# pengsongyou/openscene

Measured on AMD Instinct MI355X. Metric: active voxels/sec MinkUNet18A fwd+bwd @2cm ScanNet; per-point query ms, higher is better.
Workload: dtype f32 (bf16x6 split-precision MFMA, fp32 accumulate); 1 GPU; ScanNet distillation step (configs[2]): MinkUNet18A, 768-d head, 1 synthetic S100k scene/GPU (100999 voxels on rank 0, 2 cm), training-mode BN; timed = coordinate+kernel maps, forward, cosine loss, backward, gradient all-reduce, Adam step; arch=MinkUNet18A, feature_dim=768, voxels_rank0=100999, parallelism=dp1

## Files before the change

### include/openscene_amd.h

```cpp
#ifndef OPENSCENE_AMD_H
#define OPENSCENE_AMD_H

#include <stddef.h>
#include <stdint.h>

#ifdef __cplusplus
extern "C" {
#endif

#define OSN_OK 0
#define OSN_E_ARG (-1)
#define OSN_E_HIP (-2)
#define OSN_E_WS (-3)
#define OSN_E_RANGE (-4)

typedef void* osn_stream_t;

int osn_version(void);
const char* osn_last_error(void);
int osn_device_ok(void);

int64_t osn_hash_capacity(int64_t n);
size_t osn_coords_unique_ws_bytes(int64_t n);

// ... 60 lines not shown
int osn_spconv_fwd_tl_pc(const float* in, int64_t n_in, const void* Wp, const void* tl, const int32_t* out_rows,
                         float* out, double* bn_partial, int64_t n_out, int K, int cin, int cout, int bm,
                         void* ws, size_t ws_bytes, int32_t* counters, osn_stream_t stream);

enum { OSN_PREP_X6 = 0, OSN_PREP_TL = 1 };
typedef struct osn_prep_job {
    const float* W;
    void* out;
    int64_t first_block;
    int32_t K, cin, cout;
    int32_t flip;
    int32_t for_dgrad;
    int32_t layout;
} osn_prep_job;
int64_t osn_weight_prep_job_blocks(int K, int cin, int cout, int for_dgrad, int layout);
int osn_weight_prep_batch(const osn_prep_job* jobs_dev, int n_jobs, int64_t total_blocks, osn_stream_t stream);

int osn_spconv_fwd_plan(int64_t n_out, int K, int cin, int cout, int32_t* plan6);

int osn_stem_conv_ok(int K, int cin, int cout);
int osn_spconv_fwd_tl_ok(int64_t n_in, int K, int cin, int cout);
int osn_dense_fwd_ok(int cin, int cout);
int osn_spconv_fwd_x6_ok(int64_t n_out, int K, int cin, int cout);

int osn_weight_transpose(const float* W, int K, int cin, int cout, int flip, float* Wt,
                         osn_stream_t stream);

size_t osn_spconv_wgrad_ws_bytes(int64_t n_out, int K, int cin, int cout);
size_t osn_spconv_wgrad_items_bytes(int64_t n_out, int K, int cin, int cout);
int osn_spconv_wgrad_plan(const int64_t* counts, int64_t n_out, int K, int cin, int cout,
                          int32_t* items , osn_stream_t stream);
int osn_spconv_wgrad(const float* in, const float* gout, const int32_t* nbr, const int64_t* counts,
                     const int32_t* plan_items, float* gW, int64_t n_out, int K, int cin, int cout,
                     void* ws, size_t ws_bytes, osn_stream_t stream);

size_t osn_pair_lists_bytes(int64_t n_out, int K, int bm);
int osn_pair_lists_build(const void* tl, const int32_t* out_rows, int64_t n_out, int K, int bm, void* pl,
                         osn_stream_t stream);
size_t osn_spconv_wgrad_tl_ws_bytes(int K, int cin, int cout);
int osn_spconv_wgrad_tl(const float* in, const float* gout, const void* pl, int swap, float* gW, int64_t n_in,
                        int64_t n_out, int K, int cin, int cout, void* ws, size_t ws_bytes, osn_stream_t stream);

typedef struct osn_wgrad_job {
    const float* partial;
    const void* range;
    float* gW;
// ... 386 lines not shown
```

### openscene_amd/_lib.py

```python
import ctypes
import os
import threading

_HERE = os.path.dirname(os.path.abspath(__file__))
LIB_PATH = os.environ.get("OSN_LIB_PATH") or os.path.join(_HERE, "lib", "libopenscene_amd.so")

_c = ctypes
_vp, _i32, _i64, _sz, _f32 = _c.c_void_p, _c.c_int, _c.c_int64, _c.c_size_t, _c.c_float

PROTOTYPES = {
    "osn_version": (_i32, []),
    "osn_last_error": (_c.c_char_p, []),
    "osn_device_ok": (_i32, []),
    "osn_hash_capacity": (_i64, [_i64]),
    "osn_coords_unique_ws_bytes": (_sz, [_i64]),
    "osn_coords_unique": (_i32, [_vp, _i64, _i32, _vp, _vp, _i64, _vp, _vp, _vp, _c.POINTER(_i64), _vp, _sz, _vp]),
    "osn_coords_unique_async": (_i32, [_vp, _i64, _vp, _i32, _vp, _vp, _i64, _vp, _vp, _vp, _vp, _vp, _vp, _sz, _vp]),
    "osn_coords_pyramid_async": (_i32, [_vp, _i64, _vp, _i32, _vp, _vp, _i64, _vp, _vp, _vp, _vp, _vp, _sz, _vp]),
    "osn_kmap_build": (_i32, [_vp, _vp, _i64, _vp, _i64, _i32, _i32, _vp, _vp, _vp]),
    "osn_kmap_build_self": (_i32, [_vp, _vp, _i64, _vp, _i64, _i32, _i32, _vp, _vp, _vp]),
    "osn_kmap_transpose": (_i32, [_vp, _i64, _i32, _i64, _vp, _vp]),
    "osn_kmap_sort_ws_bytes": (_sz, [_i64]),
    "osn_kmap_sort": (_i32, [_vp, _i64, _i32, _vp, _vp, _vp, _vp, _vp, _sz, _vp]),
    "osn_kmap_count": (_i32, [_vp, _i64, _i32, _vp, _vp]),
    "osn_spconv_fwd_ws_bytes": (_sz, [_i64, _i32, _i32, _i32]),
    "osn_spconv_fwd": (_i32, [_vp, _vp, _vp, _vp, _vp, _vp, _i64, _i32, _i32, _i32, _vp, _sz, _vp]),
    "osn_weight_prep_x6_bytes": (_sz, [_i32, _i32, _i32, _i32]),
    "osn_weight_prep_x6": (_i32, [_vp, _i32, _i32, _i32, _i32, _i32, _vp, _vp]),
    "osn_weight_prep_x6_pair": (_i32, [_vp, _i32, _i32, _i32, _i32, _vp, _vp, _vp]),
    "osn_spconv_fwd_x6": (_i32, [_vp, _vp, _vp, _vp, _vp, _vp, _i64, _i32, _i32, _i32, _vp, _sz, _vp]),
    "osn_spconv_fwd_plan": (_i32, [_i64, _i32, _i32, _i32, _c.POINTER(_i32)]),
    "osn_stem_conv_ok": (_i32, [_i32, _i32, _i32]),
    "osn_spconv_fwd_tl_ok": (_i32, [_i64, _i32, _i32, _i32]),
    "osn_dense_fwd_ok": (_i32, [_i32, _i32]),
    "osn_spconv_fwd_x6_ok": (_i32, [_i64, _i32, _i32, _i32]),
    "osn_tile_rows": (_i32, [_i64]),
    "osn_tile_lists_bytes": (_sz, [_i64, _i32, _i32]),
    "osn_tile_lists_build": (_i32, [_vp, _i64, _i32, _i32, _vp, _vp]),
    "osn_weight_prep_tl_bytes": (_sz, [_i32, _i32, _i32, _i32]),
    "osn_weight_prep_tl": (_i32, [_vp, _i32, _i32, _i32, _i32, _vp, _vp, _vp]),
    "osn_weight_prep_job_blocks": (_i64, [_i32, _i32, _i32, _i32, _i32]),
    "osn_weight_prep_batch": (_i32, [_vp, _i32, _i64, _vp]),
    "osn_spconv_fwd_tl_ws_bytes": (_sz, [_i64, _i32, _i32, _i32]),
    "osn_spconv_fwd_tl": (_i32, [_vp, _i64, _vp, _vp, _vp, _vp, _vp, _i64, _i32, _i32, _i32, _i32, _vp, _sz, _vp]),
    "osn_spconv_fwd_tl_pc": (_i32, [_vp, _i64, _vp, _vp, _vp, _vp, _vp, _i64, _i32, _i32, _i32, _i32, _vp, _sz, _vp, _vp]),
    "osn_weight_transpose": (_i32, [_vp, _i32, _i32, _i32, _i32, _vp, _vp]),
    "osn_spconv_wgrad_ws_bytes": (_sz, [_i64, _i32, _i32, _i32]),
    "osn_spconv_wgrad_items_bytes": (_sz, [_i64, _i32, _i32, _i32]),
    "osn_spconv_wgrad_plan": (_i32, [_vp, _i64, _i32, _i32, _i32, _vp, _vp]),
    "osn_spconv_wgrad": (_i32, [_vp, _vp, _vp, _vp, _vp, _vp, _i64, _i32, _i32, _i32, _vp, _sz, _vp]),
    "osn_pair_lists_bytes": (_sz, [_i64, _i32, _i32]),
    "osn_pair_lists_build": (_i32, [_vp, _vp, _i64, _i32, _i32, _vp, _vp]),
    "osn_spconv_wgrad_tl_ws_bytes": (_sz, [_i32, _i32, _i32]),
    "osn_spconv_wgrad_tl": (_i32, [_vp, _vp, _vp, _i32, _vp, _i64, _i64, _i32, _i32, _i32, _vp, _sz, _vp]),
    "osn_distill_loss_state_bytes": (_sz, [_i64, _i64]),
    "osn_distill_loss_fwd": (_i32, [_vp, _vp, _vp, _i64, _i64, _i32, _i32, _vp, _vp, _sz, _vp]),
    "osn_distill_loss_bwd": (_i32, [_vp, _vp, _vp, _i64, _i64, _i32, _i32, _vp, _vp, _sz, _vp]),
    "osn_distill_loss_bwd_rows": (_i32, [_vp, _vp, _vp, _i64, _i64, _i32, _i32, _vp, _vp, _vp, _sz, _vp]),
# ... 171 lines not shown
```

### openscene_amd/csrc/spconv_tl.hip

```cpp
#include "common.h"
#include <atomic>
#include <type_traits>
#include "weight_prep.h"
#include "split.h"
#include "epilogue.h"

namespace osn {

constexpr int TL_BMAX = 88;
constexpr int TL_LIST_BMAX = 128;
constexpr int TL_BMIN = 32;
constexpr int TL_BOCC3 = 64;
constexpr int TL_LCAP = 1024;
constexpr int TL_STEPS = TL_LCAP / 32 * 4;
constexpr int TL_KMAX = 128;
constexpr int TL_CIN_MAX = TL_STEPS / (TL_LCAP / 32) * 128;
constexpr int64_t TL_ROWS_MAX = int64_t(1) << 24;
constexpr int TL_SLOTS = 512;
constexpr int TL_MAX_DEVICES = 64;

struct TlView {
    int32_t* cnt;
    int2* lst;
    int64_t nt;
    size_t bytes;
};

static TlView tl_view(const void* base, int64_t n_out, int K, int bm) {
    TlView v;
    char* p = static_cast<char*>(const_cast<void*>(base));
    v.nt = cdiv(n_out > 0 ? n_out : 1, bm);
    const size_t cb = align_up(size_t(v.nt) * K * 4, 256);
    v.cnt = reinterpret_cast<int32_t*>(p);
    v.lst = reinterpret_cast<int2*>(p ? p + cb : nullptr);
    v.bytes = cb + size_t(v.nt) * K * bm * 8;
    return v;
}

__global__ __launch_bounds__(256) void tile_lists_kernel(const int32_t* __restrict__ nbr, int64_t n_out, int K, int bm,
                                                         int32_t* __restrict__ cnt, int2* __restrict__ lst) {
    const int lane = threadIdx.x & 63, wave = threadIdx.x >> 6;
    const int64_t tile = blockIdx.x;
// ... 24 lines not shown
}

#define TL_TICK(slot)                                              \
    if (PROF) {                                                    \
        __builtin_amdgcn_sched_barrier(0);                         \
        const long long now_ = __builtin_amdgcn_s_memtime();       \
        tacc[slot] += now_ - tlast;                                \
        tlast = now_;                                              \
        __builtin_amdgcn_sched_barrier(0);                         \
    }

template <int NW, int KS, bool RAGGED, bool PROF = false, int OCC = 2, bool BUFG = false, bool EPI = false>
__global__ __launch_bounds__(256, OCC) void spconv_tl_kernel(const float* __restrict__ in, const bf16x8* __restrict__ Wp,
                                                               const int32_t* __restrict__ cnt, const int2* __restrict__ lst,
                                                               const int32_t* __restrict__ out_rows, float* __restrict__ out,
                                                               double* __restrict__ bn_partial, int32_t* __restrict__ counter,
                                                               float* __restrict__ partial, int nz, int n_out, int K, int cin,
                                                               int cout, int bm, int n_tiles, int ns, int ncb,
                                                               int self_reset, long long* __restrict__ prof, unsigned in_bytes,
                                                               const Epi epi) {
    static_assert(!(BUFG && RAGGED), "the buffer gather is for full channel chunks");
    constexpr int NT = 256;
    constexpr int CW = 32 * NW;
    constexpr int S = CW + 4;
    constexpr int CK = 32 * KS;
    constexpr int LDA = CK + 8;
    constexpr int QPR = CK / 4;
    constexpr int NQ = (32 * QPR + NT - 1) / NT;
    constexpr int NL = (TL_LCAP + NT - 1) / NT;
    extern __shared__ __attribute__((aligned(16))) float otile[];
    __shared__ __attribute__((aligned(16))) __bf16 stage[3][32][LDA];
    __shared__ uint32_t plist[TL_LCAP];
    __shared__ int klist[TL_KMAX];
    __shared__ int kcnt[TL_KMAX];
    __shared__ int lstart[TL_KMAX + 1];
    __shared__ unsigned char gowner[TL_LCAP / 32];
    __shared__ uint4 stab[TL_STEPS];
    __shared__ int nact_s, bend_s, tile_s;

    long long tacc[10] = {0, 0, 0, 0, 0, 0, 0, 0, 0, 0};
    long long tlast = PROF ? __builtin_amdgcn_s_memtime() : 0;

    const int tid = threadIdx.x, lane = tid & 63;
    const int wave = __builtin_amdgcn_readfirstlane(tid >> 6);
    const int col0 = blockIdx.y * CW;
    const int cw = wave;
    const int cb0 = blockIdx.y * (2 * NW) + 2 * cw;

    int q_row[NQ], q_col[NQ];
#pragma unroll
    for (int j = 0; j < NQ; ++j) {
        const int idx = tid + NT * j;
        q_row[j] = (idx / QPR) & 31;
        q_col[j] = (idx % QPR) * 4;
    }
    const __amdgpu_buffer_rsrc_t insrc = __builtin_amdgcn_make_buffer_rsrc(const_cast<float*>(in), 0, int(BUFG ? in_bytes : 0u), 0x00020000);
    const unsigned cin4 = unsigned(cin) * 4u;

    bf16x8 B[KS][2][3];
    float4 P0[NQ], P1[NQ];
    constexpr bool ragged = RAGGED;
    uint32_t boff[2];
#pragma unroll
    for (int nb = 0; nb < 2; ++nb) boff[nb] = (cb0 + nb < ncb ? unsigned(cb0 + nb) : 0u) * 1024u + 16u * unsigned(lane);
    const uint32_t plane_bytes = unsigned(K) * unsigned(ns) * unsigned(ncb) * 1024u;
    const uint32_t kstep_bytes = unsigned(ncb) * 1024u;
    const __amdgpu_buffer_rsrc_t wrsrc =
        __builtin_amdgcn_make_buffer_rsrc(const_cast<bf16x8*>(Wp), 0, int(3u * plane_bytes), 0x00020000);

    for (;;) {
        if (tid == 0) tile_s = atomicAdd(&counter[blockIdx.y], 1);
        __syncthreads();
        const int draw = __builtin_amdgcn_readfirstlane(tile_s);
        if (draw >= n_tiles * nz) break;
        const int tile = n_tiles - 1 - draw / nz;
        const int zpart = draw - (draw / nz) * nz;
        const int row0 = tile * bm;
        const int rows = min(bm, n_out - row0);
// ... 133 lines not shown
                }
            };
            bool b_ahead = false;
            auto step = [&](const Step& it, float4 (&P)[NQ], const Step& n1s, const Step& nf) {
                bf16x4 p1[NQ], p2[NQ], p3[NQ];
#pragma unroll
                for (int j = 0; j < NQ; ++j) {
                    float4 v = P[j];
                    if (ragged && !(32 * it.s0() + q_col[j] < cin)) v = make_float4(0.f, 0.f, 0.f, 0.f);
                    tl_split4(v, p1[j], p2[j], p3[j]);
                }
                TL_TICK(2)
                if (it.first() && !b_ahead && cw < NW) {
#pragma unroll
                    for (int ks = 0; ks < KS; ++ks) load_b(ks, it);
                }
                const bool ahead = n1s.valid() && n1s.first() && cw < NW;
                TL_TICK(8)
                __syncthreads();
                TL_TICK(3)
#pragma unroll
                for (int j = 0; j < NQ; ++j) {
                    if (NT * NQ == 32 * QPR || tid + NT * j < 32 * QPR) {
                        *reinterpret_cast<bf16x4*>(&stage[0][q_row[j]][q_col[j]]) = p1[j];
                        *reinterpret_cast<bf16x4*>(&stage[1][q_row[j]][q_col[j]]) = p2[j];
                        *reinterpret_cast<bf16x4*>(&stage[2][q_row[j]][q_col[j]]) = p3[j];
                    }
                }
                if (nf.valid()) fetch(nf, P);
                TL_TICK(9)
                __syncthreads();
                TL_TICK(4)
                if (cw >= NW) { b_ahead = false; return; }
                const bool half1 = it.np() > 16;
                const int pbase = it.base + (lane & 15);
                int ocell[2];
                f32x4 acc[2][2];
#pragma unroll
                for (int h = 0; h < 2; ++h) {
                    if (h == 0 || half1) {
                        ocell[h] = int(plist[pbase + 16 * h] >> 24) * S + 32 * cw + 4 * (lane >> 4);
                        const f32x4* cell = reinterpret_cast<const f32x4*>(__builtin_assume_aligned(&otile[ocell[h]], 16));
#pragma unroll
                        for (int nb = 0; nb < 2; ++nb) acc[h][nb] = cell[4 * nb];
                    }
                }
                const int akq = 8 * (lane >> 4);
#pragma unroll
                for (int ks = 0; ks < KS; ++ks) {
                    if (!ragged || it.s0() + ks < ns) {
                        bf16x8 af[2][3];
#pragma unroll
                        for (int h = 0; h < 2; ++h)
#pragma unroll
                            for (int pl = 0; pl < 3; ++pl)
                                af[h][pl] = *reinterpret_cast<const bf16x8*>(&stage[pl][(half1 ? h : 0) * 16 + (lane & 15)][ks * 32 + akq]);
                        auto mfma_half = [&](int h, auto ap, auto bp) {
#pragma unroll
                            for (int nb = 0; nb < 2; ++nb)
                                acc[h][nb] = __builtin_amdgcn_mfma_f32_16x16x32_bf16(B[ks][nb][bp], af[h][ap], acc[h][nb], 0, 0, 0);
                        };
                        if (half1) split_products([&](auto ap, auto bp) { mfma_half(0, ap, bp); mfma_half(1, ap, bp); });
                        else split_products([&](auto ap, auto bp) { mfma_half(0, ap, bp); });
                    }
                    if (ahead) load_b(ks, n1s);
                }
                b_ahead = ahead;
                if (PROF) {
                    float sink = 0.f;
#pragma unroll
                    for (int h = 0; h < 2; ++h)
#pragma unroll
                        for (int nb = 0; nb < 2; ++nb)
                            if (h == 0 || half1) sink += acc[h][nb][0];
                    asm volatile("" ::"v"(sink));
                }
                TL_TICK(5)
#pragma unroll
                for (int h = 0; h < 2; ++h) {
                    if (h == 0 || half1) {
                        f32x4* cell = reinterpret_cast<f32x4*>(__builtin_assume_aligned(&otile[ocell[h]], 16));
#pragma unroll
                        for (int nb = 0; nb < 2; ++nb) cell[4 * nb] = acc[h][nb];
                    }
                }
                TL_TICK(6)
            };

            Step cur = entry(0), n1 = entry(1), n2 = entry(2);
            int tn = 3;
            if (cur.valid()) fetch(cur, P0);
            if (n1.valid()) fetch(n1, P1);
            while (cur.valid()) {
                step(cur, P0, n1, n2);
                cur = n1; n1 = n2; n2 = entry(tn++);
                if (!cur.valid()) break;
                step(cur, P1, n1, n2);
                cur = n1; n1 = n2; n2 = entry(tn++);
            }
            a0 = a1;
        }
        if (park && tid < rows) orow_s[tid] = orow_pre;
        __syncthreads();

        constexpr int V = CW / 4;
        if constexpr (EPI) {
            constexpr int RPP = NT / V;
            const int c4 = tid % V, col = col0 + 4 * c4;
            if (tid < RPP * V && col < cout) {
                const EpiCols ec = epi_cols(epi, col);
                for (int j = tid / V; j < rows; j += RPP) {
                    const float4 v = *reinterpret_cast<const float4*>(&otile[j * S + 4 * c4]);
                    const int64_t orow = park ? orow_s[j] : (out_rows ? out_rows[row0 + j] : row0 + j);
                    *reinterpret_cast<float4*>(out + orow * cout + col) = epi_apply(epi, ec, v, orow, col, cout);
                }
            }
        } else
        for (int idx = tid; idx < rows * V; idx += NT) {
            const int j = idx / V, c4 = idx - j * V;
            const int col = col0 + 4 * c4;
            if (col < cout) {
                const float4 v = *reinterpret_cast<const float4*>(&otile[j * S + 4 * c4]);
                if (nz > 1) {
                    *reinterpret_cast<float4*>(partial + (int64_t(zpart) * n_out + row0 + j) * cout + col) = v;
                } else {
                    const int64_t orow = park ? orow_s[j] : (out_rows ? out_rows[row0 + j] : row0 + j);
                    *reinterpret_cast<float4*>(out + orow * cout + col) = v;
                }
            }
        }
        if (bn_partial) {
            for (int c = tid; c < CW; c += NT) {
                if (col0 + c < cout) {
                    double s1 = 0, s2 = 0;
                    for (int j = 0; j < rows; ++j) {
                        const double v = otile[j * S + c];
                        s1 += v;
                        s2 += v * v;
                    }
                    bn_partial[(int64_t(tile) * 2 + 0) * cout + col0 + c] = s1;
                    bn_partial[(int64_t(tile) * 2 + 1) * cout + col0 + c] = s2;
                }
            }
        }
        __syncthreads();
        TL_TICK(7)
    }
    if (PROF && tid == 0 && blockIdx.y == 0)
        for (int i = 0; i < 10; ++i) prof[int64_t(blockIdx.x) * 10 + i] = tacc[i];
    if ((self_reset & 1) && tid == 0) {
        const int done = atomicAdd(&counter[64 + blockIdx.y], 1);
        if (done == int(gridDim.x) - 1) {
            counter[blockIdx.y] = 0;
            counter[64 + blockIdx.y] = 0;
        }
    }
}
#undef TL_TICK

// ... 74 lines not shown
    return 512 + (nz > 1 ? size_t(nz) * size_t(n_out) * size_t(cout) * 4 : 0);
}

template <bool EPI>
__global__ void tl_reduce_parts_kernel(const float4* __restrict__ partial, int S, int64_t n_out, int c4,
                                       const int32_t* __restrict__ out_rows, float4* __restrict__ out, const Epi epi) {
    const int64_t total = n_out * c4;
    for (int64_t e = int64_t(blockIdx.x) * blockDim.x + threadIdx.x; e < total; e += int64_t(gridDim.x) * blockDim.x) {
        float4 s = partial[e];
        for (int z = 1; z < S; ++z) {
            const float4 v = partial[int64_t(z) * total + e];
            s.x += v.x; s.y += v.y; s.z += v.z; s.w += v.w;
        }
        const int64_t r = e / c4, c = e - r * c4;
        const int64_t orow = out_rows ? int64_t(out_rows[r]) : r;
        if constexpr (EPI) s = epi_quad(epi, s, orow, int(4 * c), 4 * c4);
        out[orow * c4 + c] = s;
    }
}

extern "C" int osn_spconv_fwd_tl_ok(int64_t n_in, int K, int cin, int cout) {
    return K >= 1 && K <= TL_KMAX && cin >= 8 && cin <= TL_CIN_MAX && (cin & 3) == 0 && cout >= 4 && (cout & 3) == 0 && n_in >= 0 &&
           n_in <= TL_ROWS_MAX;
}

static int spconv_fwd_tl_impl(const float* in, int64_t n_in, const void* Wp, const void* tl, const int32_t* out_rows,
                              float* out, double* bn_partial, int64_t n_out, int K, int cin, int cout, int bm, void* ws,
                              size_t ws_bytes, int32_t* counters, long long* prof, osn_stream_t stream, const Epi& epi = epi_none()) {
    hipStream_t st = static_cast<hipStream_t>(stream);
    OSN_REQUIRE(n_out >= 0 && n_out < (int64_t(1) << 31), OSN_E_ARG, "osn_spconv_fwd_tl: n_out out of range");
    OSN_REQUIRE(K >= 1 && K <= TL_KMAX && cin >= 4 && (cin & 3) == 0 && cout >= 4 && (cout & 3) == 0, OSN_E_ARG,
                "osn_spconv_fwd_tl: needs K <= %d, cin %% 4 == 0, cout %% 4 == 0 (K=%d cin=%d cout=%d)", TL_KMAX, K, cin, cout);
    OSN_REQUIRE(bm >= 1 && bm <= TL_BMAX, OSN_E_ARG, "osn_spconv_fwd_tl: bm=%d (at most %d rows per tile)", bm, TL_BMAX);
    OSN_REQUIRE(n_in >= 0 && n_in <= TL_ROWS_MAX, OSN_E_RANGE,
                "osn_spconv_fwd_tl: %lld input rows (the kernel packs an input row into 24 bits; use osn_spconv_fwd_x6)", (long long)n_in);
    if (n_out == 0) return OSN_OK;
    OSN_REQUIRE(in && Wp && out, OSN_E_ARG, "osn_spconv_fwd_tl: null pointer");
    OSN_REQUIRE(tl || (K == 1 && !out_rows), OSN_E_ARG, "osn_spconv_fwd_tl: tile lists may be null only for K == 1 (identity map)");
    OSN_REQUIRE(aligned16(in) && aligned16(Wp) && aligned16(out), OSN_E_ARG, "osn_spconv_fwd_tl: pointers must be 16-byte aligned");
    const int nw = tl_waves(cout);
    const int gy = int(cdiv(cout, 32 * nw));
    const int nz = tl ? tl_split(n_out, K, cout, bm) : 1;
    const size_t need = osn_spconv_fwd_tl_ws_bytes(n_out, tl ? K : 1, cout, bm);
    OSN_REQUIRE(ws && ws_bytes >= need && gy <= 64, OSN_E_WS, "osn_spconv_fwd_tl: workspace %zu < %zu (or more than 64 column groups)", ws_bytes, need);
    OSN_REQUIRE(!(bn_partial && nz > 1), OSN_E_ARG, "osn_spconv_fwd_tl: bn_partial is not available on split (small-table) launches");
    int32_t* counter = counters;
// ... 2 lines not shown
        counter = static_cast<int32_t*>(ws);
    }
    const int self_reset = counters ? 1 : 0;
    float* partial = reinterpret_cast<float*>(static_cast<char*>(ws) + 512);
    const int32_t* cnt = nullptr;
    const int2* lst = nullptr;
    const int64_t n_tiles = cdiv(n_out, bm);
    if (tl) {
        TlView v = tl_view(tl, n_out, K, bm);
        cnt = v.cnt; lst = v.lst;
    }
    const int ns = (cin + 31) / 32, ncb = (cout + 15) / 16;
    const int64_t units = n_tiles * nz;
    unsigned gx = unsigned(units < TL_SLOTS ? units : TL_SLOTS);
    dim3 grid(gx, unsigned(gy));
    const bf16x8* wp = static_cast<const bf16x8*>(Wp);
    const int ks = ns <= 4 ? ns : (ns % 4 == 0 ? 4 : (ns % 3 == 0 ? 3 : 4));
    OSN_REQUIRE(cdiv(ns, ks) * (TL_LCAP / 32) <= TL_STEPS, OSN_E_RANGE,
                "osn_spconv_fwd_tl: %d input channels need more than %d channel chunks per list batch (the kernel's step table); "
                "use osn_dense_fwd (K == 1) or osn_spconv_fwd_x6", cin, TL_STEPS / (TL_LCAP / 32));
    const bool ragged = (cin & 31) != 0 || ns % ks != 0;
    const bool ragged_host = ragged;
    const int ks_host = ks;
    const size_t tile_bytes = size_t(bm + 1) * size_t(32 * nw + 4) * 4;
    const bool occ3 = !prof && !ragged_host && nw <= 3 && ks_host <= 3 && tile_bytes + 28 * 1024 <= 54 * 1024;
    const uint64_t in_bytes64 = uint64_t(n_in) * uint64_t(cin) * 4u;
    const bool bufg = !prof && !ragged_host && in_bytes64 < (uint64_t(1) << 31) && n_in < (int64_t(1) << 24) && int64_t(4) * cin < (int64_t(1) << 24);
    const unsigned in_bytes = bufg ? unsigned(in_bytes64) : 0u;
    int rc_attr = OSN_OK;
    int dev_id = 0;
    OSN_HIP(hipGetDevice(&dev_id));
    const bool dev_slot_ok = dev_id >= 0 && dev_id < TL_MAX_DEVICES;
    const int dev_slot = dev_slot_ok ? dev_id : 0;
    if (occ3) {
        gx = unsigned(units < TL_SLOTS / 2 * 3 ? units : TL_SLOTS / 2 * 3);
        grid = dim3(gx, unsigned(gy));
    }
    const bool use_epi = epi.mean != nullptr && nz == 1;
#define OSN_TL4(NW_, KS_, RG_, PF_, OC_) OSN_TL5(NW_, KS_, RG_, PF_, OC_, false)
#define OSN_TL5(NW_, KS_, RG_, PF_, OC_, BG_)                                                                              \
    do {                                                                                                                   \
        if (use_epi) OSN_TL6(NW_, KS_, RG_, PF_, OC_, BG_, true);                                                          \
        else OSN_TL6(NW_, KS_, RG_, PF_, OC_, BG_, false);                                                                 \
    } while (0)
#define OSN_TL6(NW_, KS_, RG_, PF_, OC_, BG_, EP_)                                                                         \
    do {                                                                                                                   \
        auto kern = spconv_tl_kernel<NW_, KS_, RG_, PF_, OC_, BG_, EP_>;                                                   \
               \
        static std::atomic<unsigned char> attr_set[TL_MAX_DEVICES];                                                        \
        if (tile_bytes > 36 * 1024 && !(dev_slot_ok && attr_set[dev_slot].load(std::memory_order_relaxed))) {              \
            if (hipFuncSetAttribute(reinterpret_cast<const void*>(kern), hipFuncAttributeMaxDynamicSharedMemorySize,       \
                                    int(size_t(TL_BMAX + 1) * size_t(32 * NW_ + 4) * 4)) != hipSuccess) {                  \
                rc_attr = OSN_E_HIP;                                                                                       \
                break;                                                                                                     \
            }                                                                                                              \
            if (dev_slot_ok) attr_set[dev_slot].store(1, std::memory_order_relaxed);                                       \
        }                                                                                                                  \
        hipLaunchKernelGGL(kern, grid, dim3(256), tile_bytes, st, in, wp, cnt, lst, out_rows, out, bn_partial, counter, partial, nz, \
                           int(n_out), K, cin, cout, bm, int(n_tiles), ns, ncb, self_reset, prof, in_bytes,                \
                           use_epi ? epi : epi_none());                                                                    \
    } while (0)
#define OSN_TL3(NW_, KS_, RG_, PF_) OSN_TL4(NW_, KS_, RG_, PF_, 2)
#define OSN_TL2(NW_, KS_)                                                                                                  \
    do {                                                                                                                   \
        if (prof) {                                                                                                        \
            if (ragged) OSN_TL3(NW_, KS_, true, true);                                                                     \
            else OSN_TL3(NW_, KS_, false, true);                                                                           \
        } else if (ragged) {                                                                                               \
            OSN_TL3(NW_, KS_, true, false);                                                                                \
        } else if (occ3 && NW_ <= 3 && KS_ <= 3) {                                                                         \
            if (bufg) OSN_TL5((NW_ <= 3 ? NW_ : 3), (KS_ <= 3 ? KS_ : 3), false, false, 3, true);                          \
            else OSN_TL4((NW_ <= 3 ? NW_ : 3), (KS_ <= 3 ? KS_ : 3), false, false, 3);                                     \
        } else {                                                                                                           \
            if (bufg) OSN_TL5(NW_, KS_, false, false, 2, true);                                                            \
            else OSN_TL3(NW_, KS_, false, false);                                                                          \
// ... 66 lines not shown
```

### openscene_amd/csrc/spconv_ws.hip

```cpp
#include "common.h"
#include "split.h"
#include "pairlist.h"
#include "epilogue.h"

namespace osn {

constexpr int WS_NG = 4;
constexpr int WS_CH = 32 * WS_NG;

template <int NW, int KS, bool EPI = false>
__global__ __launch_bounds__(256) void spconv_ws_kernel(const float* __restrict__ in, const bf16x8* __restrict__ Wp,
                                                        const int32_t* __restrict__ gsrc, const int32_t* __restrict__ gdst,
                                                        const int32_t* __restrict__ poff, float* __restrict__ partial,
                                                        float* __restrict__ zeros, int n_dst, int K, int cin, int cout, int ns, int ncb, int chunk,
                                                        int direct, const Epi epi) {
    constexpr int NT = 256;
    constexpr int CK = 32 * KS;
    constexpr int LDA = CK + 8;
    constexpr int QPR = CK / 4;
    constexpr int NQ = (32 * QPR + NT - 1) / NT;
    __shared__ __attribute__((aligned(16))) __bf16 stage[2][3][32][LDA];
    __shared__ int sidx[WS_CH], didx[WS_CH];

    const int tid = threadIdx.x, lane = tid & 63;
    const int wave = __builtin_amdgcn_readfirstlane(tid >> 6);
    const int k = blockIdx.y;
    if (blockIdx.x == 0 && blockIdx.y == 0 && blockIdx.z == 0 && tid < 64) zeros[tid] = 0.f;
    const int pk0 = poff[k], pk1 = poff[k + 1];
    const int p0 = pk0 + blockIdx.x * chunk;
    if (p0 >= pk1) return;
    const int np = min(chunk, pk1 - p0);
    const int nsteps = (np + 31) >> 5;
    const int col0 = blockIdx.z * (32 * NW);
    const int cb0 = blockIdx.z * (2 * NW) + 2 * wave;

    for (int e = tid; e < WS_CH; e += NT) {
        sidx[e] = e < np ? gsrc[p0 + e] : 0;
        didx[e] = e < np ? gdst[p0 + e] : -1;
    }
    int q_row[NQ], q_col[NQ];
#pragma unroll
    for (int j = 0; j < NQ; ++j) {
        const int idx = tid + NT * j;
        q_row[j] = (idx / QPR) & 31;
        q_col[j] = (idx % QPR) * 4;
    }
    __syncthreads();

    f32x4 acc[WS_NG][2][2];
#pragma unroll
    for (int g = 0; g < WS_NG; ++g)
#pragma unroll
        for (int h = 0; h < 2; ++h)
#pragma unroll
            for (int nb = 0; nb < 2; ++nb) acc[g][h][nb] = f32x4{0.f, 0.f, 0.f, 0.f};

    float4 P[NQ];
    auto fetch = [&](int g, int s0) {
#pragma unroll
        for (int j = 0; j < NQ; ++j) {
            const unsigned row = unsigned(sidx[32 * g + q_row[j]]);
            const int ch = 32 * s0 + q_col[j];
            const unsigned cu = ch < cin ? unsigned(ch) : 0u;
            P[j] = *reinterpret_cast<const float4*>(in + (uint64_t(row) * unsigned(cin) + cu));
        }
    };
    int buf = 0;
    for (int s0 = 0; s0 < ns; s0 += KS) {
        bf16x8 B[KS][2][3];
// ... 1 lines not shown
#pragma unroll
            for (int ks = 0; ks < KS; ++ks)
#pragma unroll
                for (int nb = 0; nb < 2; ++nb) {
                    const bool on = s0 + ks < ns && cb0 + nb < ncb;
                    const unsigned sb = on ? unsigned(s0 + ks) : 0u, cb = on ? unsigned(cb0 + nb) : 0u;
#pragma unroll
                    for (int pl = 0; pl < 3; ++pl) {
                        const unsigned blk = (unsigned(pl * K + k) * unsigned(ns) + sb) * unsigned(ncb) + cb;
                        B[ks][nb][pl] = (Wp + (size_t(blk) << 6))[lane];
                    }
                }
        }
        fetch(0, s0);
#pragma unroll
        for (int g = 0; g < WS_NG; ++g) {
            if (g < nsteps) {
#pragma unroll
                for (int j = 0; j < NQ; ++j) {
                    const bool ok = 32 * s0 + q_col[j] < cin;
                    bf16x4 p1, p2, p3;
                    tl_split4(ok ? P[j] : make_float4(0.f, 0.f, 0.f, 0.f), p1, p2, p3);
                    if (NT * NQ == 32 * QPR || tid + NT * j < 32 * QPR) {
                        *reinterpret_cast<bf16x4*>(&stage[buf][0][q_row[j]][q_col[j]]) = p1;
                        *reinterpret_cast<bf16x4*>(&stage[buf][1][q_row[j]][q_col[j]]) = p2;
                        *reinterpret_cast<bf16x4*>(&stage[buf][2][q_row[j]][q_col[j]]) = p3;
                    }
                }
                if (g + 1 < nsteps) fetch(g + 1, s0);
                __syncthreads();
                if (wave < NW) {
                    const bool half1 = np - 32 * g > 16;
                    const int akq = 8 * (lane >> 4);
#pragma unroll
                    for (int ks = 0; ks < KS; ++ks) {
                        if (s0 + ks < ns) {
                            bf16x8 af[2][3];
#pragma unroll
                            for (int h = 0; h < 2; ++h)
#pragma unroll
                                for (int pl = 0; pl < 3; ++pl)
                                    af[h][pl] = *reinterpret_cast<const bf16x8*>(
                                        &stage[buf][pl][(half1 ? h : 0) * 16 + (lane & 15)][ks * 32 + akq]);
                            auto mfma_half = [&](int h, auto ap, auto bp) {
#pragma unroll
                                for (int nb = 0; nb < 2; ++nb)
                                    acc[g][h][nb] = __builtin_amdgcn_mfma_f32_16x16x32_bf16(B[ks][nb][bp], af[h][ap], acc[g][h][nb], 0, 0, 0);
                            };
                            if (half1) split_products([&](auto ap, auto bp) { mfma_half(0, ap, bp); mfma_half(1, ap, bp); });
                            else split_products([&](auto ap, auto bp) { mfma_half(0, ap, bp); });
                        }
                    }
                }
                buf ^= 1;
            }
        }
    }
    if (wave >= NW) return;
    EpiCols ec[2];
    if constexpr (EPI) {
#pragma unroll
        for (int nb = 0; nb < 2; ++nb) {
            const int col = col0 + 32 * wave + 16 * nb + 4 * (lane >> 4);
            ec[nb] = epi_cols(epi, col < cout ? col : 0);
        }
    }
// ... 161 lines not shown
```

### openscene_amd/csrc/wgrad_tl.hip

```cpp
#include "common.h"
#include "split.h"
#include <cstdlib>
#include "pairlist.h"

namespace osn {

typedef short s16x4 __attribute__((ext_vector_type(4)));

__device__ inline int wave_incl_scan_i32(int v, int lane) {
#pragma unroll
    for (int d = 1; d < 64; d <<= 1) {
        const int t = __shfl_up(v, d, 64);
        if (lane >= d) v += t;
    }
    return v;
}

__global__ __launch_bounds__(256) void pair_prefix_kernel(const int32_t* __restrict__ cnt, int n_tiles, int K,
                                                          int32_t* __restrict__ pref, int32_t* __restrict__ total) {
    __shared__ int wtot[4];
    __shared__ int carry_s;
    const int k = blockIdx.x, tid = threadIdx.x, lane = tid & 63, wave = tid >> 6;
    if (tid == 0) carry_s = 0;
    __syncthreads();
    for (int t0 = 0; t0 < n_tiles; t0 += 256) {
        const int t = t0 + tid;
// ... 74 lines not shown
    __syncthreads();
    if (tid < K) range[tid] = make_int2(start[tid], start[tid + 1]);
    for (int t = tid; t < PL_ITEMS; t += 256) {
        int4 it = make_int4(-1, 0, 0, 0);
        if (t < start[K]) {
            int k = 0;
            while (k + 1 < K && start[k + 1] <= t) ++k;
            const int j = t - start[k];
            it.x = k;
            it.y = j * quota;
            it.z = min(it.y + quota, total[k]);
        }
        items[t] = it;
    }
}

template <int MB, int NB, bool BUFG = false>
__global__ __launch_bounds__(256, 2) void wgrad_tl_kernel(const float* __restrict__ rows_a, const float* __restrict__ rows_g,
                                                          const int32_t* __restrict__ idx_a, const int32_t* __restrict__ idx_g,
                                                          const int32_t* __restrict__ poff, const int4* __restrict__ items,
                                                          float* __restrict__ partial, int ca, int cg, int n_cgb,
                                                          int ident_rows, int ident_quota, unsigned a_bytes, unsigned g_bytes) {
    constexpr int CA_T = 32 * MB, CG_T = 32 * NB;
    constexpr int LDA = CA_T + 8, LDG = CG_T + 8;
    constexpr int QA = CA_T / 4, QG = CG_T / 4;
    __shared__ __attribute__((aligned(16))) __bf16 Ap[3][32][LDA];
    __shared__ __attribute__((aligned(16))) __bf16 Gp[3][32][LDG];
    __shared__ int idxbuf[2][32];

    const int tid = threadIdx.x, lane = tid & 63;
    const int wave = __builtin_amdgcn_readfirstlane(tid >> 6);
    const int wi = wave >> 1, wj = wave & 1;
    const int a0 = (blockIdx.x / n_cgb) * CA_T;
    const int g0 = (blockIdx.x % n_cgb) * CG_T;
    int k, p0, p1, base;
    int pstep = 32;
    if (idx_a) {
        const int4 it = items[blockIdx.y];
        k = it.x; p0 = it.y; p1 = it.z;
        if (k < 0) return;
        base = poff[k];
        const int n_it = it.w >> 16;
        if (n_it > 1) { p0 += 32 * (it.w & 0xFFFF); pstep = 32 * n_it; }
        if (p0 >= p1) p1 = p0;
    } else {
        k = 0; base = 0;
        p0 = blockIdx.y * ident_quota;
        p1 = min(p0 + ident_quota, ident_rows);
        if (p0 >= p1) return;
    }
    (void)k;

    f32x4 acc[MB][NB];
#pragma unroll
    for (int i = 0; i < MB; ++i)
#pragma unroll
        for (int j = 0; j < NB; ++j) acc[i][j] = f32x4{0.f, 0.f, 0.f, 0.f};

    int ar[MB], ac[MB], gr[NB], gc[NB];
#pragma unroll
    for (int j = 0; j < MB; ++j) { const int idx = tid + 256 * j; ar[j] = idx / QA; ac[j] = (idx - ar[j] * QA) * 4; }
#pragma unroll
    for (int j = 0; j < NB; ++j) { const int idx = tid + 256 * j; gr[j] = idx / QG; gc[j] = (idx - gr[j] * QG) * 4; }

    const __amdgpu_buffer_rsrc_t arsrc = __builtin_amdgcn_make_buffer_rsrc(const_cast<float*>(rows_a), 0, int(BUFG ? a_bytes : 0u), 0x00020000);
    const __amdgpu_buffer_rsrc_t grsrc = __builtin_amdgcn_make_buffer_rsrc(const_cast<float*>(rows_g), 0, int(BUFG ? g_bytes : 0u), 0x00020000);
    const unsigned ca4 = unsigned(ca) * 4u, cg4 = unsigned(cg) * 4u;
    float4 pa[MB], pg[NB];
    auto load_idx = [&](int p) -> int {
        const int q = p + (tid & 31);
        if (tid >= 64) return -1;
        if (q >= p1) return -1;
        if (!idx_a) return q;
        return tid < 32 ? idx_a[base + q] : idx_g[base + q];
    };
    auto fetch = [&](int par) {
#pragma unroll
        for (int j = 0; j < MB; ++j) {
            const int r = idxbuf[0][ar[j]];
            const int ch = a0 + ac[j];
            if constexpr (BUFG) {
                pa[j] = __builtin_bit_cast(float4, __builtin_amdgcn_raw_buffer_load_b128(
                                                       arsrc, __umul24(unsigned(max(r, 0)), ca4) + 4u * unsigned(ch), 0, 0));
                continue;
            }
            const bool ok = r >= 0 && ch < ca;
// ... 22 lines not shown
    int ireg = load_idx(p0);
    if (tid < 64) idxbuf[tid >> 5][tid & 31] = ireg;
    __syncthreads();
    bool ok_a[MB], ok_g[NB];
    auto valid_now = [&]() {
#pragma unroll
        for (int j = 0; j < MB; ++j) ok_a[j] = idxbuf[0][ar[j]] >= 0 && a0 + ac[j] < ca;
#pragma unroll
        for (int j = 0; j < NB; ++j) ok_g[j] = idxbuf[1][gr[j]] >= 0 && g0 + gc[j] < cg;
    };
    valid_now();
    fetch(0);
    ireg = load_idx(p0 + pstep);

    for (int p = p0; p < p1; p += pstep) {
        bf16x4 a1[MB], a2[MB], a3[MB], g1[NB], g2[NB], g3[NB];
#pragma unroll
        for (int j = 0; j < MB; ++j) split4(pa[j], ok_a[j], a1[j], a2[j], a3[j]);
#pragma unroll
        for (int j = 0; j < NB; ++j) split4(pg[j], ok_g[j], g1[j], g2[j], g3[j]);
        __syncthreads();
#pragma unroll
        for (int j = 0; j < MB; ++j) {
            *reinterpret_cast<bf16x4*>(&Ap[0][ar[j]][ac[j]]) = a1[j];
            *reinterpret_cast<bf16x4*>(&Ap[1][ar[j]][ac[j]]) = a2[j];
            *reinterpret_cast<bf16x4*>(&Ap[2][ar[j]][ac[j]]) = a3[j];
        }
#pragma unroll
        for (int j = 0; j < NB; ++j) {
            *reinterpret_cast<bf16x4*>(&Gp[0][gr[j]][gc[j]]) = g1[j];
            *reinterpret_cast<bf16x4*>(&Gp[1][gr[j]][gc[j]]) = g2[j];
            *reinterpret_cast<bf16x4*>(&Gp[2][gr[j]][gc[j]]) = g3[j];
        }
        if (tid < 64) idxbuf[tid >> 5][tid & 31] = ireg;
        __syncthreads();
        if (p + pstep < p1) {
            valid_now();
            fetch(0);
            ireg = load_idx(p + 2 * pstep);
        }
        const int li = lane & 15, lg = lane >> 4;
        auto frag = [&](const __bf16* plane, int pitch, int c16) -> bf16x8 {
            const __bf16* q = plane + (8 * lg + (li >> 2)) * pitch + c16 + 4 * (li & 3);
            const s16x4 lo = __builtin_amdgcn_ds_read_tr16_b64_v4i16(
                (__attribute__((address_space(3))) s16x4*)(q));
            const s16x4 hi = __builtin_amdgcn_ds_read_tr16_b64_v4i16(
                (__attribute__((address_space(3))) s16x4*)(q + 4 * pitch));
            union { s16x4 h[2]; bf16x8 v; } u;
            u.h[0] = lo; u.h[1] = hi;
            return u.v;
        };
        bf16x8 fa[MB][3], fg[NB][3];
#pragma unroll
        for (int i = 0; i < MB; ++i)
#pragma unroll
            for (int pl = 0; pl < 3; ++pl) fa[i][pl] = frag(&Ap[pl][0][0], LDA, (wi * MB + i) * 16);
#pragma unroll
        for (int j = 0; j < NB; ++j)
#pragma unroll
            for (int pl = 0; pl < 3; ++pl) fg[j][pl] = frag(&Gp[pl][0][0], LDG, (wj * NB + j) * 16);
#pragma unroll
        for (int i = 0; i < MB; ++i)
#pragma unroll
            for (int j = 0; j < NB; ++j) {
                f32x4 t = acc[i][j];
                split_products([&](auto ap, auto gp) {
                    t = __builtin_amdgcn_mfma_f32_16x16x32_bf16(fa[i][ap], fg[j][gp], t, 0, 0, 0);
                });
                acc[i][j] = t;
            }
// ... 268 lines not shown
```

Measured before the change: 13.01 million voxels/s.

## Swizzle LDS staging layouts to cut bank conflicts and padding in conv kernels

Adds a shared LDS layout header and routes the forward tile-list, workspace and wgrad kernels through it. For 32- and 96-wide chunks the forward A staging buffer drops its row padding and uses an XOR swizzle instead. The wgrad staging uses a wider pitch (c+16) and a permuted row order for the transposed reads, both meant to avoid LDS bank conflicts. The occupancy-3 check now uses a real per-CU LDS budget with allocation granules. It also adds a query API exposing the layouts. The risks are subtle indexing bugs, and the larger wgrad pitch may reduce occupancy.

```diff
diff --git a/include/openscene_amd.h b/include/openscene_amd.h
--- a/include/openscene_amd.h
+++ b/include/openscene_amd.h
@@ -106,6 +106,12 @@
 int osn_spconv_fwd_tl_ok(int64_t n_in, int K, int cin, int cout);
 int osn_dense_fwd_ok(int cin, int cout);
 int osn_spconv_fwd_x6_ok(int64_t n_out, int K, int cin, int cout);
+
+#define OSN_LDS_TL_ROWS 0
+#define OSN_LDS_TL_TILE 1
+#define OSN_LDS_WGRAD_ROWS 2
+#define OSN_LDS_WS_ROWS 3
+int osn_lds_layout(int family, int channels, int32_t* out34);
 
 int osn_weight_transpose(const float* W, int K, int cin, int cout, int flip, float* Wt,
                          osn_stream_t stream);
diff --git a/openscene_amd/_lib.py b/openscene_amd/_lib.py
--- a/openscene_amd/_lib.py
+++ b/openscene_amd/_lib.py
@@ -34,6 +34,7 @@
     "osn_spconv_fwd_tl_ok": (_i32, [_i64, _i32, _i32, _i32]),
     "osn_dense_fwd_ok": (_i32, [_i32, _i32]),
     "osn_spconv_fwd_x6_ok": (_i32, [_i64, _i32, _i32, _i32]),
+    "osn_lds_layout": (_i32, [_i32, _i32, _vp]),
     "osn_tile_rows": (_i32, [_i64]),
     "osn_tile_lists_bytes": (_sz, [_i64, _i32, _i32]),
     "osn_tile_lists_build": (_i32, [_vp, _i64, _i32, _i32, _vp, _vp]),
diff --git a/openscene_amd/csrc/lds_layout.h b/openscene_amd/csrc/lds_layout.h
--- /dev/null
+++ b/openscene_amd/csrc/lds_layout.h
@@ -0,0 +1,28 @@
+#pragma once
+
+namespace osn {
+namespace lds {
+
+constexpr bool tl_rows_swizzled(int ck) { return ck == 32 || ck == 96; }
+constexpr bool ws_rows_swizzled(int) { return false; }
+constexpr int conv_a_pitch(int ck, bool swz) { return swz ? ck : ck + 8; }
+constexpr int conv_a_xor(bool swz, int row) { return swz ? (4 - ((row >> 2) & 3)) & 3 : 0; }
+constexpr int conv_a_at(int ck, bool swz, int row, int col) {
+    return row * conv_a_pitch(ck, swz) + (((col >> 3) ^ conv_a_xor(swz, row)) << 3) + (col & 7);
+}
+constexpr int conv_a_col_at(bool swz, int row, int pos) { return ((((pos >> 1) ^ conv_a_xor(swz, row)) << 1) | (pos & 1)) << 2; }
+static_assert(conv_a_at(96, true, 13, conv_a_col_at(true, 13, 7)) == 13 * 96 + 4 * 7 && conv_a_at(32, true, 6, conv_a_col_at(true, 6, 5)) == 6 * 32 + 4 * 5,
+              "a swizzled row has no padding: quad position pos of row r is element 4 (r ck / 4 + pos) of the plane");
+
+constexpr int conv_tile_stride(int cw) { return cw + 4; }
+constexpr int conv_tile_at(int cw, int row, int chunk) { return row * conv_tile_stride(cw) + 4 * chunk; }
+
+constexpr int wgrad_pitch(int c) { return c + 16; }
+constexpr int wgrad_row(int pair) { return (pair & ~12) | ((pair & 4) << 1) | ((pair & 8) >> 1); }
+
+constexpr int LDS_PER_CU = 160 * 1024;
+constexpr int LDS_GRANULE = 1280;
+constexpr int lds_alloc(int bytes) { return (bytes + LDS_GRANULE - 1) / LDS_GRANULE * LDS_GRANULE; }
+
+}
+}
diff --git a/openscene_amd/csrc/spconv_tl.hip b/openscene_amd/csrc/spconv_tl.hip
--- a/openscene_amd/csrc/spconv_tl.hip
+++ b/openscene_amd/csrc/spconv_tl.hip
@@ -4,6 +4,7 @@
 #include "weight_prep.h"
 #include "split.h"
 #include "epilogue.h"
+#include "lds_layout.h"
 
 namespace osn {
 
@@ -18,6 +19,9 @@
 constexpr int64_t TL_ROWS_MAX = int64_t(1) << 24;
 constexpr int TL_SLOTS = 512;
 constexpr int TL_MAX_DEVICES = 64;
+constexpr int TL_LDS_TABLES = TL_LCAP * 4 + 2 * TL_KMAX * 4 + (TL_KMAX + 1) * 4 + TL_LCAP / 32 + TL_STEPS * 16 + 3 * 4;
+constexpr int tl_lds_static(int ks) { return 3 * 32 * lds::conv_a_pitch(32 * ks, lds::tl_rows_swizzled(32 * ks)) * 2 + TL_LDS_TABLES; }
+constexpr int tl_lds_tile(int nw, int bm) { return (bm + 1) * lds::conv_tile_stride(32 * nw) * 4; }
 
 struct TlView {
     int32_t* cnt;
@@ -88,14 +92,15 @@
     static_assert(!(BUFG && RAGGED), "the buffer gather is for full channel chunks");
     constexpr int NT = 256;
     constexpr int CW = 32 * NW;
-    constexpr int S = CW + 4;
+    constexpr int S = lds::conv_tile_stride(CW);
     constexpr int CK = 32 * KS;
-    constexpr int LDA = CK + 8;
+    constexpr bool SWZ = lds::tl_rows_swizzled(CK);
+    constexpr int LDA = lds::conv_a_pitch(CK, SWZ);
     constexpr int QPR = CK / 4;
     constexpr int NQ = (32 * QPR + NT - 1) / NT;
     constexpr int NL = (TL_LCAP + NT - 1) / NT;
     extern __shared__ __attribute__((aligned(16))) float otile[];
-    __shared__ __attribute__((aligned(16))) __bf16 stage[3][32][LDA];
+    __shared__ __attribute__((aligned(16))) __bf16 stage[3][32 * LDA];
     __shared__ uint32_t plist[TL_LCAP];
     __shared__ int klist[TL_KMAX];
     __shared__ int kcnt[TL_KMAX];
@@ -118,8 +123,10 @@
     for (int j = 0; j < NQ; ++j) {
         const int idx = tid + NT * j;
         q_row[j] = (idx / QPR) & 31;
-        q_col[j] = (idx % QPR) * 4;
-    }
+        q_col[j] = lds::conv_a_col_at(SWZ, q_row[j], idx % QPR);
+    }
+    const int a_at = lds::conv_a_at(CK, SWZ, lane & 15, 8 * (lane >> 4));
+    const int o_chunk = 8 * cw + (lane >> 4);
     const __amdgpu_buffer_rsrc_t insrc = __builtin_amdgcn_make_buffer_rsrc(const_cast<float*>(in), 0, int(BUFG ? in_bytes : 0u), 0x00020000);
     const unsigned cin4 = unsigned(cin) * 4u;
 
@@ -299,9 +306,10 @@
 #pragma unroll
                 for (int j = 0; j < NQ; ++j) {
                     if (NT * NQ == 32 * QPR || tid + NT * j < 32 * QPR) {
-                        *reinterpret_cast<bf16x4*>(&stage[0][q_row[j]][q_col[j]]) = p1[j];
-                        *reinterpret_cast<bf16x4*>(&stage[1][q_row[j]][q_col[j]]) = p2[j];
-                        *reinterpret_cast<bf16x4*>(&stage[2][q_row[j]][q_col[j]]) = p3[j];
+                        const int at = SWZ ? 4 * (tid + NT * j) : lds::conv_a_at(CK, SWZ, q_row[j], q_col[j]);
+                        *reinterpret_cast<bf16x4*>(&stage[0][at]) = p1[j];
+                        *reinterpret_cast<bf16x4*>(&stage[1][at]) = p2[j];
+                        *reinterpret_cast<bf16x4*>(&stage[2][at]) = p3[j];
                     }
                 }
                 if (nf.valid()) fetch(nf, P);
@@ -316,13 +324,13 @@
 #pragma unroll
                 for (int h = 0; h < 2; ++h) {
                     if (h == 0 || half1) {
-                        ocell[h] = int(plist[pbase + 16 * h] >> 24) * S + 32 * cw + 4 * (lane >> 4);
-                        const f32x4* cell = reinterpret_cast<const f32x4*>(__builtin_assume_aligned(&otile[ocell[h]], 16));
-#pragma unroll
-                        for (int nb = 0; nb < 2; ++nb) acc[h][nb] = cell[4 * nb];
+                        const int orow = int(plist[pbase + 16 * h] >> 24);
+                        ocell[h] = lds::conv_tile_at(CW, orow, o_chunk);
+#pragma unroll
+                        for (int nb = 0; nb < 2; ++nb)
+                            acc[h][nb] = *reinterpret_cast<const f32x4*>(__builtin_assume_aligned(&otile[ocell[h] + 16 * nb], 16));
                     }
                 }
-                const int akq = 8 * (lane >> 4);
 #pragma unroll
                 for (int ks = 0; ks < KS; ++ks) {
                     if (!ragged || it.s0() + ks < ns) {
@@ -331,7 +339,8 @@
                         for (int h = 0; h < 2; ++h)
 #pragma unroll
                             for (int pl = 0; pl < 3; ++pl)
-                                af[h][pl] = *reinterpret_cast<const bf16x8*>(&stage[pl][(half1 ? h : 0) * 16 + (lane & 15)][ks * 32 + akq]);
+                                af[h][pl] = *reinterpret_cast<const bf16x8*>(
+                                    &stage[pl][(half1 ? h : 0) * 16 * LDA + a_at + 32 * ks]);
                         auto mfma_half = [&](int h, auto ap, auto bp) {
 #pragma unroll
                             for (int nb = 0; nb < 2; ++nb)
@@ -356,9 +365,9 @@
 #pragma unroll
                 for (int h = 0; h < 2; ++h) {
                     if (h == 0 || half1) {
-                        f32x4* cell = reinterpret_cast<f32x4*>(__builtin_assume_aligned(&otile[ocell[h]], 16));
-#pragma unroll
-                        for (int nb = 0; nb < 2; ++nb) cell[4 * nb] = acc[h][nb];
+#pragma unroll
+                        for (int nb = 0; nb < 2; ++nb)
+                            *reinterpret_cast<f32x4*>(__builtin_assume_aligned(&otile[ocell[h] + 16 * nb], 16)) = acc[h][nb];
                     }
                 }
                 TL_TICK(6)
@@ -387,7 +396,7 @@
             if (tid < RPP * V && col < cout) {
                 const EpiCols ec = epi_cols(epi, col);
                 for (int j = tid / V; j < rows; j += RPP) {
-                    const float4 v = *reinterpret_cast<const float4*>(&otile[j * S + 4 * c4]);
+                    const float4 v = *reinterpret_cast<const float4*>(&otile[lds::conv_tile_at(CW, j, c4)]);
                     const int64_t orow = park ? orow_s[j] : (out_rows ? out_rows[row0 + j] : row0 + j);
                     *reinterpret_cast<float4*>(out + orow * cout + col) = epi_apply(epi, ec, v, orow, col, cout);
                 }
@@ -397,7 +406,7 @@
             const int j = idx / V, c4 = idx - j * V;
             const int col = col0 + 4 * c4;
             if (col < cout) {
-                const float4 v = *reinterpret_cast<const float4*>(&otile[j * S + 4 * c4]);
+                const float4 v = *reinterpret_cast<const float4*>(&otile[lds::conv_tile_at(CW, j, c4)]);
                 if (nz > 1) {
                     *reinterpret_cast<float4*>(partial + (int64_t(zpart) * n_out + row0 + j) * cout + col) = v;
                 } else {
@@ -411,7 +420,7 @@
                 if (col0 + c < cout) {
                     double s1 = 0, s2 = 0;
                     for (int j = 0; j < rows; ++j) {
-                        const double v = otile[j * S + c];
+                        const double v = otile[lds::conv_tile_at(CW, j, c >> 2) + (c & 3)];
                         s1 += v;
                         s2 += v * v;
                     }
@@ -532,6 +541,34 @@
 extern "C" int osn_spconv_fwd_tl_ok(int64_t n_in, int K, int cin, int cout) {
     return K >= 1 && K <= TL_KMAX && cin >= 8 && cin <= TL_CIN_MAX && (cin & 3) == 0 && cout >= 4 && (cout & 3) == 0 && n_in >= 0 &&
            n_in <= TL_ROWS_MAX;
+}
+
+extern "C" int osn_lds_layout(int family, int channels, int32_t* out34) {
+    OSN_REQUIRE(out34, OSN_E_ARG, "osn_lds_layout: null pointer");
+    OSN_REQUIRE(channels == 32 || channels == 64 || channels == 96 || channels == 128, OSN_E_ARG,
+                "osn_lds_layout: channels=%d (the kernels' chunks are 32, 64, 96 or 128 wide)", channels);
+    switch (family) {
+        case OSN_LDS_TL_ROWS:
+        case OSN_LDS_WS_ROWS: {
+            const bool swz = family == OSN_LDS_TL_ROWS ? lds::tl_rows_swizzled(channels) : lds::ws_rows_swizzled(channels);
+            out34[0] = lds::conv_a_pitch(channels, swz) * 2;
+            out34[1] = family == OSN_LDS_TL_ROWS ? tl_lds_static(channels / 32) : 2 * 3 * 32 * out34[0] + 2 * 128 * 4;
+            for (int r = 0; r < 32; ++r) out34[2 + r] = lds::conv_a_xor(swz, r);
+            return OSN_OK;
+        }
+        case OSN_LDS_TL_TILE:
+            out34[0] = lds::conv_tile_stride(channels) * 4;
+            out34[1] = tl_lds_tile(channels / 32, TL_BOCC3);
+            for (int r = 0; r < 32; ++r) out34[2 + r] = 0;
+            return OSN_OK;
+        case OSN_LDS_WGRAD_ROWS:
+            out34[0] = lds::wgrad_pitch(channels) * 2;
+            out34[1] = 3 * 32 * lds::wgrad_pitch(channels) * 2;
+            for (int r = 0; r < 32; ++r) out34[2 + r] = lds::wgrad_row(r);
+            return OSN_OK;
+        default: break;
+    }
+    OSN_REQUIRE(false, OSN_E_ARG, "osn_lds_layout: family=%d", family);
 }
 
 static int spconv_fwd_tl_impl(const float* in, int64_t n_in, const void* Wp, const void* tl, const int32_t* out_rows,
@@ -580,8 +617,9 @@
     const bool ragged = (cin & 31) != 0 || ns % ks != 0;
     const bool ragged_host = ragged;
     const int ks_host = ks;
-    const size_t tile_bytes = size_t(bm + 1) * size_t(32 * nw + 4) * 4;
-    const bool occ3 = !prof && !ragged_host && nw <= 3 && ks_host <= 3 && tile_bytes + 28 * 1024 <= 54 * 1024;
+    const size_t tile_bytes = size_t(tl_lds_tile(nw, bm));
+    const bool occ3 = !prof && !ragged_host && nw <= 3 && ks_host <= 3 &&
+                      3 * lds::lds_alloc(tl_lds_static(ks_host) + int(tile_bytes)) <= lds::LDS_PER_CU;
     const uint64_t in_bytes64 = uint64_t(n_in) * uint64_t(cin) * 4u;
     const bool bufg = !prof && !ragged_host && in_bytes64 < (uint64_t(1) << 31) && n_in < (int64_t(1) << 24) && int64_t(4) * cin < (int64_t(1) << 24);
     const unsigned in_bytes = bufg ? unsigned(in_bytes64) : 0u;
@@ -608,7 +646,7 @@
         static std::atomic<unsigned char> attr_set[TL_MAX_DEVICES];                                                        \
         if (tile_bytes > 36 * 1024 && !(dev_slot_ok && attr_set[dev_slot].load(std::memory_order_relaxed))) {              \
             if (hipFuncSetAttribute(reinterpret_cast<const void*>(kern), hipFuncAttributeMaxDynamicSharedMemorySize,       \
-                                    int(size_t(TL_BMAX + 1) * size_t(32 * NW_ + 4) * 4)) != hipSuccess) {                  \
+                                    tl_lds_tile(NW_, TL_BMAX)) != hipSuccess) {                  \
                 rc_attr = OSN_E_HIP;                                                                                       \
                 break;                                                                                                     \
             }                                                                                                              \
diff --git a/openscene_amd/csrc/spconv_ws.hip b/openscene_amd/csrc/spconv_ws.hip
--- a/openscene_amd/csrc/spconv_ws.hip
+++ b/openscene_amd/csrc/spconv_ws.hip
@@ -2,6 +2,7 @@
 #include "split.h"
 #include "pairlist.h"
 #include "epilogue.h"
+#include "lds_layout.h"
 
 namespace osn {
 
@@ -16,10 +17,11 @@
                                                         int direct, const Epi epi) {
     constexpr int NT = 256;
     constexpr int CK = 32 * KS;
-    constexpr int LDA = CK + 8;
+    constexpr bool SWZ = lds::ws_rows_swizzled(CK);
+    constexpr int LDA = lds::conv_a_pitch(CK, SWZ);
     constexpr int QPR = CK / 4;
     constexpr int NQ = (32 * QPR + NT - 1) / NT;
-    __shared__ __attribute__((aligned(16))) __bf16 stage[2][3][32][LDA];
+    __shared__ __attribute__((aligned(16))) __bf16 stage[2][3][32 * LDA];
     __shared__ int sidx[WS_CH], didx[WS_CH];
 
     const int tid = threadIdx.x, lane = tid & 63;
@@ -43,8 +45,9 @@
     for (int j = 0; j < NQ; ++j) {
         const int idx = tid + NT * j;
         q_row[j] = (idx / QPR) & 31;
-        q_col[j] = (idx % QPR) * 4;
-    }
+        q_col[j] = lds::conv_a_col_at(SWZ, q_row[j], idx % QPR);
+    }
+    const int a_at = lds::conv_a_at(CK, SWZ, lane & 15, 8 * (lane >> 4));
     __syncthreads();
 
     f32x4 acc[WS_NG][2][2];
@@ -92,16 +95,16 @@
                     bf16x4 p1, p2, p3;
                     tl_split4(ok ? P[j] : make_float4(0.f, 0.f, 0.f, 0.f), p1, p2, p3);
                     if (NT * NQ == 32 * QPR || tid + NT * j < 32 * QPR) {
-                        *reinterpret_cast<bf16x4*>(&stage[buf][0][q_row[j]][q_col[j]]) = p1;
-                        *reinterpret_cast<bf16x4*>(&stage[buf][1][q_row[j]][q_col[j]]) = p2;
-                        *reinterpret_cast<bf16x4*>(&stage[buf][2][q_row[j]][q_col[j]]) = p3;
+                        const int at = SWZ ? 4 * (tid + NT * j) : lds::conv_a_at(CK, SWZ, q_row[j], q_col[j]);
+                        *reinterpret_cast<bf16x4*>(&stage[buf][0][at]) = p1;
+                        *reinterpret_cast<bf16x4*>(&stage[buf][1][at]) = p2;
+                        *reinterpret_cast<bf16x4*>(&stage[buf][2][at]) = p3;
                     }
                 }
                 if (g + 1 < nsteps) fetch(g + 1, s0);
                 __syncthreads();
                 if (wave < NW) {
                     const bool half1 = np - 32 * g > 16;
-                    const int akq = 8 * (lane >> 4);
 #pragma unroll
                     for (int ks = 0; ks < KS; ++ks) {
                         if (s0 + ks < ns) {
@@ -111,7 +114,7 @@
 #pragma unroll
                                 for (int pl = 0; pl < 3; ++pl)
                                     af[h][pl] = *reinterpret_cast<const bf16x8*>(
-                                        &stage[buf][pl][(half1 ? h : 0) * 16 + (lane & 15)][ks * 32 + akq]);
+                                        &stage[buf][pl][(half1 ? h : 0) * 16 * LDA + a_at + 32 * ks]);
                             auto mfma_half = [&](int h, auto ap, auto bp) {
 #pragma unroll
                                 for (int nb = 0; nb < 2; ++nb)
diff --git a/openscene_amd/csrc/wgrad_tl.hip b/openscene_amd/csrc/wgrad_tl.hip
--- a/openscene_amd/csrc/wgrad_tl.hip
+++ b/openscene_amd/csrc/wgrad_tl.hip
@@ -2,6 +2,7 @@
 #include "split.h"
 #include <cstdlib>
 #include "pairlist.h"
+#include "lds_layout.h"
 
 namespace osn {
 
@@ -122,7 +123,7 @@
                                                           float* __restrict__ partial, int ca, int cg, int n_cgb,
                                                           int ident_rows, int ident_quota, unsigned a_bytes, unsigned g_bytes) {
     constexpr int CA_T = 32 * MB, CG_T = 32 * NB;
-    constexpr int LDA = CA_T + 8, LDG = CG_T + 8;
+    constexpr int LDA = lds::wgrad_pitch(CA_T), LDG = lds::wgrad_pitch(CG_T);
     constexpr int QA = CA_T / 4, QG = CG_T / 4;
     __shared__ __attribute__((aligned(16))) __bf16 Ap[3][32][LDA];
     __shared__ __attribute__((aligned(16))) __bf16 Gp[3][32][LDG];
@@ -157,11 +158,19 @@
 #pragma unroll
         for (int j = 0; j < NB; ++j) acc[i][j] = f32x4{0.f, 0.f, 0.f, 0.f};
 
-    int ar[MB], ac[MB], gr[NB], gc[NB];
-#pragma unroll
-    for (int j = 0; j < MB; ++j) { const int idx = tid + 256 * j; ar[j] = idx / QA; ac[j] = (idx - ar[j] * QA) * 4; }
-#pragma unroll
-    for (int j = 0; j < NB; ++j) { const int idx = tid + 256 * j; gr[j] = idx / QG; gc[j] = (idx - gr[j] * QG) * 4; }
+    int ar[MB], ac[MB], gr[NB], gc[NB], a_at[MB], g_at[NB];
+#pragma unroll
+    for (int j = 0; j < MB; ++j) {
+        const int idx = tid + 256 * j;
+        ar[j] = idx / QA; ac[j] = (idx - ar[j] * QA) * 4;
+        a_at[j] = lds::wgrad_row(ar[j]) * LDA + ac[j];
+    }
+#pragma unroll
+    for (int j = 0; j < NB; ++j) {
+        const int idx = tid + 256 * j;
+        gr[j] = idx / QG; gc[j] = (idx - gr[j] * QG) * 4;
+        g_at[j] = lds::wgrad_row(gr[j]) * LDG + gc[j];
+    }
 
     const __amdgpu_buffer_rsrc_t arsrc = __builtin_amdgcn_make_buffer_rsrc(const_cast<float*>(rows_a), 0, int(BUFG ? a_bytes : 0u), 0x00020000);
     const __amdgpu_buffer_rsrc_t grsrc = __builtin_amdgcn_make_buffer_rsrc(const_cast<float*>(rows_g), 0, int(BUFG ? g_bytes : 0u), 0x00020000);
@@ -230,15 +239,15 @@
         __syncthreads();
 #pragma unroll
         for (int j = 0; j < MB; ++j) {
-            *reinterpret_cast<bf16x4*>(&Ap[0][ar[j]][ac[j]]) = a1[j];
-            *reinterpret_cast<bf16x4*>(&Ap[1][ar[j]][ac[j]]) = a2[j];
-            *reinterpret_cast<bf16x4*>(&Ap[2][ar[j]][ac[j]]) = a3[j];
+            *reinterpret_cast<bf16x4*>(&Ap[0][0][a_at[j]]) = a1[j];
+            *reinterpret_cast<bf16x4*>(&Ap[1][0][a_at[j]]) = a2[j];
+            *reinterpret_cast<bf16x4*>(&Ap[2][0][a_at[j]]) = a3[j];
         }
 #pragma unroll
         for (int j = 0; j < NB; ++j) {
-            *reinterpret_cast<bf16x4*>(&Gp[0][gr[j]][gc[j]]) = g1[j];
-            *reinterpret_cast<bf16x4*>(&Gp[1][gr[j]][gc[j]]) = g2[j];
-            *reinterpret_cast<bf16x4*>(&Gp[2][gr[j]][gc[j]]) = g3[j];
+            *reinterpret_cast<bf16x4*>(&Gp[0][0][g_at[j]]) = g1[j];
+            *reinterpret_cast<bf16x4*>(&Gp[1][0][g_at[j]]) = g2[j];
+            *reinterpret_cast<bf16x4*>(&Gp[2][0][g_at[j]]) = g3[j];
         }
         if (tid < 64) idxbuf[tid >> 5][tid & 31] = ireg;
         __syncthreads();
@@ -249,11 +258,12 @@
         }
         const int li = lane & 15, lg = lane >> 4;
         auto frag = [&](const __bf16* plane, int pitch, int c16) -> bf16x8 {
-            const __bf16* q = plane + (8 * lg + (li >> 2)) * pitch + c16 + 4 * (li & 3);
+            const int pair = 8 * lg + (li >> 2);
+            const __bf16* q = plane + lds::wgrad_row(pair) * pitch + c16 + 4 * (li & 3);
             const s16x4 lo = __builtin_amdgcn_ds_read_tr16_b64_v4i16(
                 (__attribute__((address_space(3))) s16x4*)(q));
             const s16x4 hi = __builtin_amdgcn_ds_read_tr16_b64_v4i16(
-                (__attribute__((address_space(3))) s16x4*)(q + 4 * pitch));
+                (__attribute__((address_space(3))) s16x4*)(q + lds::wgrad_row(4) * pitch));
             union { s16x4 h[2]; bf16x8 v; } u;
             u.h[0] = lo; u.h[1] = hi;
             return u.v;
```

After: 12.37 million voxels/s. 0.951x the previous value.
